# pabr/leansdr

Measured on AMD Instinct MI355X. Metric: IQ MSamples/s demodulated (leandvb QPSK 1/2), higher is better.
Workload: dtype f32; 1 GPU; BASELINE config 2: QPSK 1/2, Fs 240 MS/s cf32 (120 sps), device-resident endless stream; scaler(x75 fused) + fir_filter(N=313,D=30) + cstln_receiver(omega 4, linear sampler); fir_arith=LSDR_FIR_MFMA_BLK (f32 matrix pipe, block-polyphase; tolera…, batch_samples_per_capture=268369920, captures_per_gpu=1, rx_mode=tiled, parallelism=1 independent capture(s), 1 per GPU, no collectives, no RCCL

## Files before the change

### leansdr_amd/csrc/cstln_receiver.hip

```cpp
#include <cmath>
#include "capture_input.h"

namespace {

constexpr int kChunk = 128;
constexpr int kRrcLdsTaps = 1024;

#ifdef LSDR_RX_TRACE
__device__ unsigned long long g_rx_probe[8];
#define LSDR_RXP(i) { asm volatile("s_waitcnt vmcnt(0) lgkmcnt(0)" ::: "memory"); unsigned long long t__ = __builtin_amdgcn_s_memtime(); \
  asm volatile("s_waitcnt lgkmcnt(0)" ::: "memory"); \
  if (i > 0) rxp_acc[i] += t__ - rxp_t; else if (rxp_t) rxp_acc[4] += t__ - rxp_t; \
  if (i == 3) { rxp_acc[0] += 1; unsigned long long u__ = __builtin_amdgcn_s_memtime(); asm volatile("s_waitcnt lgkmcnt(0)" ::: "memory"); rxp_acc[5] += u__ - t__; t__ = u__; } \
  rxp_t = t__; }
#define LSDR_RXP_FLUSH { if (threadIdx.x == 0 && blockIdx.x == (gridDim.x > 1 ? 1u : 0u)) for (int k__ = 0; k__ < 6; ++k__) atomicAdd(&g_rx_probe[k__], rxp_acc[k__]); }
#else
#define LSDR_RXP(i)
#define LSDR_RXP_FLUSH
#endif
constexpr float kCstlnAmp = 75.0f;

struct __attribute__((aligned(8))) lut_entry {
  int16_t cost;
  uint8_t symbol;
// ... 430 lines not shown
        st.meas_count -= a.C.meas_decimation;
        rx_meas m; m.freqw = st.freqw; m.est_insp = st.est_insp; m.est_sp = st.est_sp; m.est_ep = st.est_ep; m.a = 0.f; m.tile = 0u;
        a.meas[sh_nm++] = m;
      }
    }
    pos += kChunk;
    __syncthreads();
    if (have_next) {
#pragma unroll
      for (int q = 0; q < 3; ++q)
        if (lane + 64 * q < span) buf[lane + 64 * q] = pre[q];
      for (int k = lane + 192; k < span; k += 64) buf[k] = src[pos + k];
    }
    __syncthreads();
  }
  if (lane == 0) {
    *a.state = st;
    a.counters[0] = pos; a.counters[1] = sh_nout; a.counters[2] = sh_nm; a.counters[3] = sh_nc;
  }
}


struct rx_state_dev;
__device__ __forceinline__ lsdr_softsymbol rx_relabel(lsdr_softsymbol v, const uint8_t *map) { v.symbol = map[v.symbol]; return v; }
__device__ __forceinline__ unsigned rx_symbol_of(lsdr_softsymbol v) { return v.symbol; }
__device__ __forceinline__ float fmod65536(float x);
__device__ __forceinline__ void rx_rotate_back(rx_state_dev *st, unsigned rot, float quad);
__device__ __forceinline__ float rx_freq_tap(const rx_state_dev *st) { return st->freqw / 65536; }
#include "rx_tiling.h"
typedef rx_tile_info_t<lsdr_softsymbol> rx_tile_info;

__device__ __forceinline__ void rx_rotate_back(rx_state_dev *st, unsigned rot, float quad) {
  st->phase = fmod65536(st->phase - rot * quad);
}

struct rx_tiled_args {
  const void *in;
  unsigned long long total_chunks;
  unsigned first_chunks, tile_chunks, warm_chunks;
  unsigned n_tiles;
  unsigned lanes_per_wave;
  unsigned dbg;
  unsigned stage_stride;
  lsdr_softsymbol *stage;
  lsdr_softsymbol *wstage;
  unsigned wstride;
  rx_tile_info *info;
  unsigned *hstage;
  unsigned long long hpitch;
  rx_tile_info_h *hinfo;
  rx_ema_map *ema;
  rx_ema_map *ema_wave;
  const rx_state_dev *state;
  rx_state_dev *state_next;
  rx_meas *meas;
  unsigned long long meas_base;
  float2 *cstln;
  rx_consts C;
  rx_tables T;
};

__device__ __forceinline__ void rx_tile_meas(const rx_tiled_args &a, unsigned long long c, unsigned tile, float freqw,
                                             const rx_ema_map &m) {
  const unsigned long long md = a.C.meas_decimation;
  const unsigned long long before = (a.meas_base + c * kChunk) / md, after = (a.meas_base + (c + 1) * kChunk) / md;
  const unsigned long long first_m = a.meas_base / md;
  for (unsigned long long q = before; q < after; ++q) {
    rx_meas mm; mm.freqw = freqw; mm.a = m.a; mm.est_insp = m.bi; mm.est_sp = m.bs; mm.est_ep = m.be; mm.tile = tile;
    a.meas[q - first_m] = mm;
  }
}

template <int SAMP, int FMT, bool HARD, bool SOFT_T = false>
__device__ __forceinline__ void rx_tile_exact(const rx_tiled_args &a, float in_scale = 1.0f, unsigned in_flip = 0u) {
  typename in_stream<FMT>::type src = in_make<FMT>(a.in);
  in_conv(src, in_scale, in_flip);
  unsigned long long c1 = a.first_chunks;
  if (c1 > a.total_chunks) c1 = a.total_chunks;
  rx_state_dev s = *a.state;
  rx_tile_info ti;
  ti.has_pre = 0; ti.pre.cost = 0; ti.pre.symbol = 0; ti.pre.pad = 0; ti.n_warm = 0;
  ti.mu_begin = s.mu; ti.phase_begin = s.phase;
  lsdr_softsymbol *po = a.stage;
  unsigned cnt = 0;
  unsigned hacc = 0, htail = 0;
  auto emit = [&](lsdr_softsymbol ss) {
    if (HARD) {
      hacc = (hacc << 2) | (ss.symbol & 3u); htail = (htail << 2) | (ss.symbol & 3u);
      if (SOFT_T) { po[(unsigned long long)cnt * a.hpitch] = ss; ++cnt; }
      else if ((++cnt & 15u) == 0) a.hstage[(unsigned long long)((cnt >> 4) - 1) * a.hpitch] = hacc;
    } else {
      po[cnt++] = ss;
    }
  };
  rx_ema_map m; m.a = 0.f; m.bi = s.est_insp; m.bs = s.est_sp; m.be = s.est_ep;
  for (unsigned long long c = 0; c < c1; ++c) {
    if (SAMP == 1) s.samp_freqw = s.freqw;
    if (SAMP == 2) {
      int ph = s.update_freq_phase - 128;
      if (ph <= 0) {
        const float f = s.freqw / a.C.subsampling;
        const int N = a.C.ncoeffs;
        for (int i = 0; i < N; ++i) {
          const float2 e = ld_uniform::expi(a.T, trig_index(-f * (i - N / 2)));
          const float cc = a.T.coeffs[i];
          a.T.shifted[i] = make_float2(e.x * cc, e.y * cc);
        }
        ph = N * 16;
      }
      s.update_freq_phase = ph;
    }
    bool wrote;
    rx_chunk<SAMP, ld_uniform>(a.T, a.C, s, src + c * kChunk, emit, a.cstln ? a.cstln + c : nullptr, &wrote);
    if (a.cstln && !wrote) a.cstln[c] = make_float2(__builtin_nanf(""), __builtin_nanf(""));
    m.bi = s.est_insp; m.bs = s.est_sp; m.be = s.est_ep;
    if (a.meas) rx_tile_meas(a, c, 0u, s.freqw, m);
  }
  ti.mu_end = s.mu; ti.phase_end = s.phase; ti.count = cnt;
  if (HARD) {
    if (!SOFT_T && (cnt & 15u)) a.hstage[(unsigned long long)(cnt >> 4) * a.hpitch] = hacc << (2 * (16 - (cnt & 15u)));
    rx_tile_info_h th;
    th.mu_begin = ti.mu_begin; th.phase_begin = ti.phase_begin; th.mu_end = ti.mu_end; th.phase_end = ti.phase_end;
    th.count = cnt; th.has_pre = 0; th.n_warm = 0; th.warm_tail = 0; th.body_tail = htail;
    a.hinfo[0] = th;
  } else {
    a.info[0] = ti;
  }
  { rx_ema_map id; id.a = 1.f; id.bi = id.bs = id.be = 0.f; a.ema[0] = id; }
  a.ema_wave[0] = m;
  if (a.n_tiles == 1) {
    s.meas_count = (a.meas_base + a.total_chunks * kChunk) % a.C.meas_decimation;
    *a.state_next = s;
  }
}

template <int FMT> struct rx_stage;
template <> struct rx_stage<LSDR_IN_CU8> {
  static constexpr int kStage = 64;
  static constexpr int kStageMargin = 16;
  static constexpr int kBps = 2;
  static constexpr int kRowBytes = kBps * (kStage + kStageMargin) + 16;
  static constexpr int kWindow = 8;
};
template <> struct rx_stage<LSDR_IN_CF32> {
  static constexpr int kStage = 16;
  static constexpr int kStageMargin = 1;
  static constexpr int kBps = 8;
  static constexpr int kRowBytes = kBps * (kStage + kStageMargin) + 8;
  static constexpr int kWindow = 16;
};
static_assert(rx_stage<LSDR_IN_CU8>::kRowBytes % 16 == 0 && rx_stage<LSDR_IN_CF32>::kRowBytes % 16 == 0, "stage geometry");
static_assert(kChunk % rx_stage<LSDR_IN_CU8>::kStage == 0 && kChunk % rx_stage<LSDR_IN_CF32>::kStage == 0, "stage geometry");
typedef __attribute__((address_space(3))) void *rx_lds_ptr;

constexpr int kEstSpan = 512;
template <typename SRC>
__device__ __forceinline__ float rx_wave_timing(const SRC &src, long long first, long long end, float omega, int lane, float *quality) {
  float cr = 0.f, sr = 0.f, pw = 0.f;
  const float w = 1.0f / omega;
#pragma unroll
  for (int i = 0; i < kEstSpan / 64; ++i) {
    const int idx = i * 64 + lane;
    if (first + idx < end) {
      const float2 x = src[first + idx];
      const float hann = 0.5f - 0.5f * __builtin_amdgcn_cosf((float)idx * (1.0f / kEstSpan));
      const float p = (x.x * x.x + x.y * x.y) * hann;
      const float rev = (float)idx * w;
      const float fr = rev - __builtin_floorf(rev);
      cr += p * __builtin_amdgcn_cosf(fr); sr += p * __builtin_amdgcn_sinf(fr); pw += p;
    }
  }
#pragma unroll
  for (int d = 32; d >= 1; d >>= 1) { cr += __shfl_xor(cr, d, 64); sr += __shfl_xor(sr, d, 64); pw += __shfl_xor(pw, d, 64); }
  *quality = pw > 0.f ? __builtin_sqrtf(cr * cr + sr * sr) / pw : 0.f;
  float rev = atan2f(sr, cr) * 0.15915494f;
  rev -= __builtin_floorf(rev);
  return rev * omega;
}

template <int SAMP, bool ARITH, int FMT, bool LDS, bool HARD>
__device__ __forceinline__ void rx_tile_tol(const rx_tiled_args &a, unsigned j0, int lane, char *lds) {
  const bool valid = lane < (int)a.lanes_per_wave && j0 + (unsigned)lane < a.n_tiles;
  const rx_consts &C = a.C;
  const bool rrc_lds = SAMP == 2 && C.ncoeffs <= kRrcLdsTaps;
  float est_first = 0.f, est_step = 0.f;
  bool est_ok = false;
  unsigned est_j0 = j0;
  if (SAMP != 2 && C.omega >= 2.0f && (a.lanes_per_wave == 32u || a.lanes_per_wave == 64u)) {
    const long long end = (long long)a.total_chunks * kChunk + (SAMP == 1 ? 1 : 0);
    const typename in_stream<FMT>::type all = in_make<FMT>(a.in);
    for (unsigned g = 0; g < a.lanes_per_wave / 32u; ++g) {
      const unsigned jf = j0 + 32u * g;
      if (jf >= a.n_tiles) break;
      const unsigned jl = jf + 31u < a.n_tiles - 1 ? jf + 31u : a.n_tiles - 1;
      const long long wsf = ((long long)a.first_chunks + (long long)(jf - 1) * a.tile_chunks - a.warm_chunks) * kChunk;
      const long long wsl = wsf + (long long)(jl - jf) * a.tile_chunks * kChunk;
      float q0 = 0.f, q1 = 0.f, step = 0.f;
      const float t0 = rx_wave_timing(all, wsf, end, C.omega, lane, &q0);
      const bool ok = q0 > 0.02f && wsf + kEstSpan <= end;
      if (ok && jl > jf && wsl + kEstSpan <= end) {
        const float t1 = rx_wave_timing(all, wsl, end, C.omega, lane, &q1);
        if (q1 > 0.02f) {
          const double span = (double)(wsl - wsf), om = (double)C.omega;
          double pred = (double)t0 - span; pred -= om * __builtin_floor(pred / om);
          float d = t1 - (float)pred;
          d -= C.omega * __builtin_rintf(d / C.omega);
          step = d / (float)(jl - jf);
        }
      }
      if ((unsigned)lane / 32u == g || a.lanes_per_wave == 32u) { est_first = t0; est_step = step; est_ok = ok; est_j0 = jf; }
    }
  }
  if (!LDS && !valid) return;
  const unsigned j = valid ? j0 + (unsigned)lane : j0;
  const unsigned long long c0 = a.first_chunks + (unsigned long long)(j - 1) * a.tile_chunks;
  unsigned long long c1 = c0 + a.tile_chunks;
  if (c1 > a.total_chunks) c1 = a.total_chunks;
  const unsigned long long cb = c0 - a.warm_chunks;
  const int nwarm = (int)a.warm_chunks, nchunks = valid ? (int)(c1 - cb) : 0;
  const int wave_chunks = LDS ? nwarm + (int)a.tile_chunks : nchunks;
  const int ra = SAMP == 1 ? 1 : (SAMP == 2 ? C.ncoeffs - 1 : 0);
  const int n_last = nchunks * kChunk - 1 + ra;
  const typename in_stream<FMT>::type base = in_make<FMT>(a.in) + cb * kChunk;

  typedef rx_stage<FMT> ST;
  constexpr int kStage = ST::kStage, kRowBytes = ST::kRowBytes, kStageLoads = ST::kRowBytes / 16;
  const char *row = nullptr;
  int delta = 0;
  __amdgpu_buffer_rsrc_t rsrc;
  unsigned src_off[LDS ? kStageLoads : 1];
  if (LDS) {
    const unsigned long long addr = (unsigned long long)a.in;
    delta = (int)(addr & 15ull);
    const unsigned long long cb0 = a.first_chunks + (unsigned long long)(j0 - 1) * a.tile_chunks - a.warm_chunks;
    const unsigned long long org = FMT == LSDR_IN_CU8 ? 0ull : cb0;
    const unsigned long long bytes = (((a.total_chunks - org) * kChunk + (unsigned)ra) * (unsigned)ST::kBps + (unsigned)delta + 15ull) & ~15ull;
    rsrc = __builtin_amdgcn_make_buffer_rsrc(const_cast<char *>(reinterpret_cast<const char *>(a.in)) + org * (kChunk * ST::kBps) - delta, 0,
                                             (int)(bytes > 0xffffffffull ? 0xffffffffu : (unsigned)bytes), 0x00020000);
    row = lds + lane * kRowBytes;
#pragma unroll
    for (int q = 0; q < kStageLoads; ++q) {
      const unsigned f = (unsigned)q * 1024u + (unsigned)lane * 16u, r = f / (unsigned)kRowBytes, col = f - r * (unsigned)kRowBytes;
      const unsigned long long tile_byte = (cb0 - org + (unsigned long long)r * a.tile_chunks) * (kChunk * (unsigned long long)ST::kBps);
      src_off[q] = (j0 + r < a.n_tiles && tile_byte + col < 0xfff00000ull) ? (unsigned)(tile_byte + col) : 0xfffffff0u;
    }
  }

  const rx_state_dev *S = a.state;
  float freqw = S->freqw, agc = S->agc_gain, est_insp = S->est_insp, est_sp = S->est_sp, est_ep = S->est_ep;
  const float min_f = S->min_freqw, max_f = S->max_freqw;
  float fwin = 65536.0f / C.omega / 2048.0f;
  if (fwin < 8.f) fwin = 8.f;
  const float f_lo = freqw - fwin, f_hi = freqw + fwin;
  float mu = 0.f, phase = 0.f;
  {
    const double ws = (double)cb * kChunk - (double)S->mu, om = (double)C.omega;
    const double r = ws - om * __builtin_floor(ws / om);
    mu = (float)(r > 0.0 ? om - r : 0.0);
    if (est_ok) {
      const double off = (double)(j - est_j0) * a.tile_chunks * kChunk;
      double t = (double)est_first + (double)est_step * (double)(j - est_j0) - off;
      t -= om * __builtin_floor(t / om);
      float dm = (float)t - mu;
      dm -= C.omega * __builtin_rintf(dm / C.omega);
      if (__builtin_fabsf(dm) > 0.33f) mu = (float)t;
    }
    if (!(mu >= 0.f && mu < C.omega)) mu = 0.f;
  }
  float h0pr = 0.f, h0pi = 0.f, h0cr = 0.f, h0ci = 0.f, h1pr = 0.f, h1pi = 0.f, h1cr = 0.f, h1ci = 0.f;
  float h2pr = 0.f, h2pi = 0.f, h2cr = 0.f, h2ci = 0.f;
  const float kk = C.kest, k1 = 1 - C.kest;
  const float acq_alpha = C.acq_alpha, freq_alpha = C.freq_alpha, acq_gain_mu = C.acq_gain_mu, gain_mu = C.gain_mu;
  const float freq_beta = C.freq_beta, omega = C.omega;
  const int acq_syms = C.acq_syms;
  rx_ema_map m; m.a = 1.f; m.bi = 0.f; m.bs = 0.f; m.be = 0.f;

  rx_tile_info ti;
  ti.has_pre = 0; ti.pre.cost = 0; ti.pre.symbol = 0; ti.pre.pad = 0; ti.n_warm = 0;
  ti.mu_begin = ti.phase_begin = 0.f;
  unsigned last = 0;
  unsigned *const po = reinterpret_cast<unsigned *>(a.stage + (unsigned long long)j * a.stage_stride);
  unsigned *const pw = reinterpret_cast<unsigned *>(a.wstage + (unsigned long long)j * a.wstride);
  unsigned *const pw0 = reinterpret_cast<unsigned *>(a.wstage + (unsigned long long)j0 * a.wstride);
  unsigned cnt = 0, got = 0;
  unsigned hacc = 0, htail = 0, hwarm = 0, hnwarm = 0, hcnt = 0;
  unsigned q0 = 0, q1 = 0, q2 = 0, q3 = 0, qn = 0;
  unsigned *bp = po;
  const bool quads = !HARD && !(a.dbg & 1u);
  unsigned *const hcol = HARD ? a.hstage + j : nullptr;

  int n = 0;
  rx_window<FMT> win;
  if (!LDS) {
    win.load(base, 0, n_last);
    if (!HARD) *pw = 0u;
  } else {
    win.wn = -16;
  }
  for (int ci = 0; ci < wave_chunks; ++ci) {
    const bool active = !LDS || ci < nchunks;
    const bool body = ci >= nwarm, lastwarm = ci + 1 == nwarm;
    const int cend = (ci + 1) * kChunk;
    if (active && ci == nwarm) {
      ti.mu_begin = mu; ti.phase_begin = phase;
      ti.pre.cost = (int16_t)(last & 0xffffu); ti.pre.symbol = (uint8_t)(last >> 16); ti.has_pre = got ? 1u : 0u;
      hwarm = htail; hnwarm = got < 16u ? got : 16u;
    }
    const float samp_freqw = freqw;
    unsigned *dp = body ? po + cnt : (lastwarm ? pw : pw0);
    unsigned keep = (body || lastwarm) ? 1u : 0u;
    if (a.dbg & 1u) { dp = pw0; keep = 0u; }
    bool had = false;
    float2 sg = make_float2(0.f, 0.f), sv = make_float2(0.f, 0.f);
    int pt_re = 0, pt_im = 0;
    unsigned nsym = 0;
    auto skip = [&]() {
      if (!(mu < 1.f)) {
        const int rem = cend - n;
        int k = (int)mu;
        if (k < 1 || k > rem) k = rem;
        mu -= (float)k; n += k; phase += (float)k * freqw;
      }
    };
    if (active) skip();
#pragma unroll 1
    for (int sb = 0; sb < (LDS ? kChunk / kStage : 1); ++sb) {
      const int s0 = ci * kChunk + sb * kStage;
      const int send = LDS ? s0 + kStage : cend;
      auto lds_window = [&](rx_window<FMT> &wd, int i) {
        int bo = ST::kBps * (i - s0) + delta;
        bo = bo < 0 ? 0 : (bo > kRowBytes - ST::kWindow ? kRowBytes - ST::kWindow : bo);
        rx_window_lds(wd, row, bo, delta, s0);
      };
      if (LDS) {
        const unsigned soff = (unsigned)__builtin_amdgcn_readfirstlane(s0 * ST::kBps);
#pragma unroll
        for (int q = 0; q < kStageLoads; ++q)
          __builtin_amdgcn_raw_ptr_buffer_load_lds(rsrc, (rx_lds_ptr)(size_t)(unsigned)(unsigned long long)(lds + q * 1024), 16, src_off[q], soff, 0, 0);
        __builtin_amdgcn_s_waitcnt(0x0F70);
        asm volatile("" ::: "memory");
        if (active && n < send && (FMT == LSDR_IN_CF32 || !win.covers(n))) lds_window(win, n);
      }
      while (active && n < send) {
        if (SAMP != 2 && !win.covers(n) && !(a.dbg & 2u)) {
          if (LDS) lds_window(win, n);
          else {
            win.load(base, n, n_last);
            __builtin_amdgcn_s_waitcnt(0x0F70);
          }
        }
        float2 p0, p1;
        win.get(n, p0, p1);
        const float2 sx0 = cmul(p0, ld_hwtrig::expi(a.T, trig_index(-phase)));
        if (SAMP == 2) {
          float2 acc = make_float2(0.f, 0.f);
          const int SS = C.subsampling, N = C.ncoeffs;
          int px = n;
          int pc = (int)((1 - mu) * SS);
          auto tap = [&](int i) -> float2 { return rrc_lds ? reinterpret_cast<const float2 *>(lds)[i] : a.T.shifted_tol[i]; };
          if (FMT == LSDR_IN_CF32) {
            for (; pc + SS < N; pc += 2 * SS, px += 2) {
              const float4 xx = *reinterpret_cast<const float4 *>(reinterpret_cast<const float2 *>(base.p) + px);
              const float2 t0 = cmul(tap(pc), make_float2(xx.x, xx.y));
              acc.x += t0.x; acc.y += t0.y;
              const float2 t1 = cmul(tap(pc + SS), make_float2(xx.z, xx.w));
              acc.x += t1.x; acc.y += t1.y;
            }
          }
          for (; pc < N; pc += SS, ++px) {
            const float2 tt = cmul(tap(pc), base[px]);
            acc.x += tt.x; acc.y += tt.y;
          }
          sg = cmul(ld_hwtrig::expi(a.T, trig_index(-phase)), acc);
        } else if (SAMP == 1) {
          const float2 sx1 = cmul(p1, ld_hwtrig::expi(a.T, trig_index(-(phase + samp_freqw))));
          const float k0 = 1 - mu;
          sg = make_float2(sx0.x * k0 + sx1.x * mu, sx0.y * k0 + sx1.y * mu);
        } else {
          sg = sx0;
        }
        sv = make_float2(sg.x * agc, sg.y * agc);
        uint2 raw;
        if (!ARITH) raw = *reinterpret_cast<const uint2 *>(a.T.lut + lut_index(sv.x, sv.y));
        int lo = (int)(mu + omega - 0.1f);
        lo = lo < 1 ? 1 : lo;
        rx_window<FMT> nxt;
        if (LDS) lds_window(nxt, n + lo);
        else if (a.dbg & 2u) { nxt = win; nxt.wn = n + lo; }
        else nxt.load(base, n + lo, n_last);
        lut_entry e;
        if (ARITH) {
          float hi = sv.x, hq = sv.y;
          lut_halve(hi, hq);
          const qpsk_decision qd = qpsk_decide((int)hi, (int)hq);
          e.cost = (int16_t)qd.cost; e.symbol = (uint8_t)qd.symbol; e.zero = 0;
          e.phase_error = (int16_t)qd.phase_error; e.pt_re = (int8_t)qd.pt_re; e.pt_im = (int8_t)qd.pt_im;
          raw.x = ((unsigned)qd.cost & 0xffffu) | (qd.symbol << 16);
        } else {
          e = lut_unpack(raw.x, raw.y);
        }
        if (HARD) {
          const unsigned hs = (raw.x >> 16) & 3u;
          htail = (htail << 2) | hs;
          if (body) {
            hacc = (hacc << 2) | hs;
            if ((++hcnt & 15u) == 0) hcol[(unsigned long long)((hcnt >> 4) - 1) * a.hpitch] = hacc;
          }
        } else if (quads && body) {
          q0 = q1; q1 = q2; q2 = q3; q3 = raw.x;
          if (++qn == 4u) {
            *reinterpret_cast<uint4 *>(bp) = make_uint4(q0, q1, q2, q3);
            bp += 4; qn = 0;
          }
        } else {
          *dp = raw.x; dp += keep;
        }
        last = raw.x;
        ++nsym;
        const bool acq = (int)(got + nsym) <= acq_syms && !body;
        phase += e.phase_error * (acq ? acq_alpha : freq_alpha);
        freqw += e.phase_error * freq_beta;
        freqw = freqw < f_lo ? f_lo : freqw; freqw = freqw > f_hi ? f_hi : freqw;
        h2pr = h1pr; h2pi = h1pi; h2cr = h1cr; h2ci = h1ci;
        h1pr = h0pr; h1pi = h0pi; h1cr = h0cr; h1ci = h0ci;
        h0pr = sv.x; h0pi = sv.y;
        pt_re = e.pt_re; pt_im = e.pt_im;
        had = true;
        h0cr = (float)pt_re; h0ci = (float)pt_im;
        const float muerr = ((h0pr - h2pr) * h1cr + (h0pi - h2pi) * h1ci) - ((h0cr - h2cr) * h1pr + (h0ci - h2ci) * h1pi);
        float mucorr = muerr * (acq ? acq_gain_mu : gain_mu);
        mucorr = mucorr < -0.1f ? -0.1f : mucorr; mucorr = mucorr > 0.1f ? 0.1f : mucorr;
        mu += mucorr;
        mu += omega;
        mu -= 1.f; phase += freqw; ++n;
        win = nxt;
        skip();
      }
    }
    if (active) {
      phase = fmod65536(phase);
      if (had) {
        const float insp = sg.x * sg.x + sg.y * sg.y;
        est_insp = insp * kk + est_insp * k1;
        if (est_insp) agc = kCstlnAmp / __builtin_sqrtf(est_insp);
        const float evr = sv.x - pt_re, evi = sv.y - pt_im;
        float sig_power, ev_power;
        if (C.nsymbols == 2) {
          const float sig_real = (float)((double)(pt_re + pt_im) * 0.707);
          const float ev_real = (float)((double)(evr + evi) * 0.707);
          sig_power = sig_real * sig_real; ev_power = ev_real * ev_real;
        } else {
          sig_power = (float)(pt_re * pt_re + pt_im * pt_im);
          ev_power = evr * evr + evi * evi;
        }
        est_sp = sig_power * kk + est_sp * k1;
        est_ep = ev_power * kk + est_ep * k1;
        if (body) {
          m.a *= k1;
          m.bi = insp * kk + m.bi * k1; m.bs = sig_power * kk + m.bs * k1; m.be = ev_power * kk + m.be * k1;
        }
      }
      if (!C.allow_drift) {
        if (freqw < min_f || freqw > max_f) freqw = (max_f + min_f) / 2;
      }
      if (body) cnt += nsym; else got += nsym;
      if (lastwarm) ti.n_warm = nsym;
      if (body && a.meas) rx_tile_meas(a, cb + (unsigned long long)ci, j, freqw, m);
      if (body && a.cstln) a.cstln[cb + (unsigned long long)ci] = had ? sv : make_float2(__builtin_nanf(""), __builtin_nanf(""));
    }
  }
  ti.mu_end = mu; ti.phase_end = phase; ti.count = cnt;
  if (quads && qn) {
    const uint4 v = qn == 1u ? make_uint4(q3, 0u, 0u, 0u) : (qn == 2u ? make_uint4(q2, q3, 0u, 0u) : make_uint4(q1, q2, q3, 0u));
    *reinterpret_cast<uint4 *>(bp) = v;
  }
  if (valid) {
    if (HARD) {
      if (hcnt & 15u) hcol[(unsigned long long)(hcnt >> 4) * a.hpitch] = hacc << (2 * (16 - (hcnt & 15u)));
      rx_tile_info_h th;
      th.mu_begin = ti.mu_begin; th.phase_begin = ti.phase_begin; th.mu_end = mu; th.phase_end = phase;
      th.count = cnt; th.has_pre = ti.has_pre; th.n_warm = hnwarm; th.warm_tail = hwarm; th.body_tail = htail;
      a.hinfo[j] = th;
    } else {
      a.info[j] = ti;
    }
  }
  {
    rx_ema_map inc = m;
    const int gl = lane & 31;
#pragma unroll
    for (int d = 1; d < 32; d <<= 1) {
      rx_ema_map o;
// ... 173 lines not shown
    nout += cnt;
    s.meas_count += kChunk;
    while (s.meas_count >= a.C.meas_decimation) s.meas_count -= a.C.meas_decimation;
  }
  if (quads && (nout & 3ull)) {
    unsigned *pu = reinterpret_cast<unsigned *>(po);
    const unsigned r = (unsigned)(nout & 3ull);
    if (r == 1u) pu[nout - 1] = q3;
    else if (r == 2u) { pu[nout - 2] = q2; pu[nout - 1] = q3; }
    else { pu[nout - 3] = q1; pu[nout - 2] = q2; pu[nout - 1] = q3; }
  }
  a.states[sidx] = s;
  a.produced[sidx] = nout;
}

#include "notch_detect.h"
#include "rxb_device.h"

}

struct lsdr_rx {
  lsdr_ctx *ctx;
  lsdr_rx_cfg cfg;
  std::vector<float> coeffs;
  lsdr::cstln_tables tabs;
  float omega, min_omega, max_omega;
  rx_state_dev st;
  rx_state_dev st_initial;
  bool st_dirty_host;
  float2 *d_trig;
  lut_entry *d_lut;
  float *d_coeffs;
  float2 *d_shifted, *d_shifted_tol;
  rx_state_dev *d_state;
  unsigned long long *d_counters;
  rx_meas *d_meas; size_t meas_cap;
  float2 *d_cstln; size_t cstln_cap;
  lsdr_softsymbol *d_stage; size_t stage_cap;
  lsdr_softsymbol *d_wstage; size_t wstage_cap;
  unsigned *d_hstage; size_t hstage_cap;
  rx_tile_info_h *d_hinfo;
  size_t out_sym_offset;
  bool time_on; hipEvent_t tev0[8], tev1[8]; bool tev_set[8]; double time_ms; unsigned time_n;
  rx_tile_info *d_info; rx_tile_fix *d_fix; size_t tiles_cap;
  rx_ema_map *d_ema;
  rx_ema_map *d_ema_wave;
  rx_state_dev *d_state_next;
  rx_state_dev *h_snap;
  static constexpr unsigned kSnapSlots = 4;
  uint8_t *d_relabel;
  struct rx_seam_result *d_seam;
  struct rx_seam_part *d_part;
  std::vector<uint8_t> relabel;
  unsigned last_tiles, last_dup, last_miss, last_badseam;
  static const int kRing = 8;
  struct rx_seam_result *h_res;
  struct rx_seam_result *h_res_dev;
  hipEvent_t ev[kRing];
  unsigned ring_tiles[kRing];
  int ring_head, ring_count;
  float retired_freq_tap;
  bool st_stale_host;
  bool qpsk_arith;
  unsigned arith_max_dpe;
};

static void rx_state_export(const rx_state_dev &s, lsdr_rx_state *st) {
  st->mu = s.mu; st->phase = s.phase; st->freqw = s.freqw; st->agc_gain = s.agc_gain;
  st->est_insp = s.est_insp; st->est_sp = s.est_sp; st->est_ep = s.est_ep;
  st->freq_tap = s.freqw / 65536;
  st->min_freqw = s.min_freqw; st->max_freqw = s.max_freqw;
  st->meas_count = s.meas_count;
  memcpy(st->hist, s.hist, sizeof(st->hist));
}

static void rx_update_freq_limits(lsdr_rx *r, bool have_cstln) {
  int n = 4;
  if (have_cstln) {
    switch (r->tabs.nsymbols) {
      case 2: n = 2; break;
      case 4: n = 4; break;
      case 8: n = 8; break;
      case 16: n = 12; break;
      case 32: n = 16; break;
      default: n = 4; break;
    }
  }
  r->st.min_freqw = r->st.freqw - 65536 / r->max_omega / n / 2;
  r->st.max_freqw = r->st.freqw + 65536 / r->max_omega / n / 2;
}
static void rx_set_omega(lsdr_rx *r, float omega, bool have_cstln) {
  float tol = (float)10e-6;
  r->omega = omega;
  r->min_omega = omega * (1 - tol);
  r->max_omega = omega * (1 + tol);
  rx_update_freq_limits(r, have_cstln);
}
static void rx_set_freq(lsdr_rx *r, float freq, bool have_cstln) {
  r->st.freqw = freq * 65536;
  rx_update_freq_limits(r, have_cstln);
}

static int rx_push_state(lsdr_rx *r) {
  if (!r->st_dirty_host) return LSDR_OK;
  LSDR_HIP(hipMemcpyAsync(r->d_state, &r->st, sizeof(rx_state_dev), hipMemcpyHostToDevice, r->ctx->stream));
  LSDR_HIP(hipStreamSynchronize(r->ctx->stream));
  r->st_dirty_host = false;
  return LSDR_OK;
}

static void rx_fill_consts(const lsdr_rx *r, rx_consts &C, rx_tables &T) {
  C.omega = r->omega;
  C.freq_alpha = (float)0.04;
  C.freq_beta = (float)(0.0012 / (double)r->omega * (double)r->cfg.pll_adjustment);
  C.gain_mu = (float)(0.02 / (double)(kCstlnAmp * kCstlnAmp) * 2);
  C.kest = r->cfg.kest;
  C.allow_drift = r->cfg.allow_drift;
  C.nsymbols = r->tabs.nsymbols;
  C.meas_decimation = r->cfg.meas_decimation;
  C.ncoeffs = r->cfg.ncoeffs;
  C.subsampling = r->cfg.subsampling;
  {
    const char *e;
    C.acq_syms = (e = getenv("LSDR_RX_ACQ_SYMS")) ? atoi(e) : 0;
    C.acq_alpha = C.freq_alpha * ((e = getenv("LSDR_RX_ACQ_ALPHA")) ? (float)atof(e) : 1.f);
    C.acq_gain_mu = C.gain_mu * ((e = getenv("LSDR_RX_ACQ_MU")) ? (float)atof(e) : 1.f);
  }
  T.trig = r->d_trig; T.lut = r->d_lut; T.coeffs = r->d_coeffs; T.shifted = r->d_shifted; T.shifted_tol = r->d_shifted_tol;
}

static int rx_pull_state(lsdr_rx *r) {
  if (!r->st_stale_host) return LSDR_OK;
  LSDR_HIP(hipMemcpyAsync(&r->st, r->d_state, sizeof(rx_state_dev), hipMemcpyDeviceToHost, r->ctx->stream));
  LSDR_HIP(hipStreamSynchronize(r->ctx->stream));
  r->st_stale_host = false;
  return LSDR_OK;
}

struct rx_plan {
  rx_tiled_args a;
  lsdr_softsymbol *out;
  size_t chunks, nm;
  unsigned n_tiles, blocks, lpw, stage_stride, sym_per_chunk;
  unsigned long long hpitch, meas_base, md;
  bool want_meas, want_cstln, use_lds, hard;
  int slot;
};

struct rx_hooks {
  bool no_lds_set; int no_lds;
  unsigned long long lds_span;
  int lanes;
  bool prio;
  unsigned dbg; bool skip;
};
static const rx_hooks &rx_env() {
  static const rx_hooks h = [] {
    rx_hooks v;
    const char *e = getenv("LSDR_RX_NO_LDS");
    v.no_lds_set = e != nullptr; v.no_lds = e ? atoi(e) : 0;
    v.lds_span = (e = getenv("LSDR_RX_LDS_SPAN")) ? strtoull(e, nullptr, 0) : 0xfff00000ull;
    v.lanes = (e = getenv("LSDR_RX_LANES")) ? atoi(e) : 0;
    v.prio = (e = getenv("LSDR_RX_PRIO")) && atoi(e);
    v.dbg = (e = LSDR_MEASURE_ENV("LSDR_RX_DBG")) ? (unsigned)atoi(e) & 3u : 0u;
    v.skip = LSDR_MEASURE_ENV("LSDR_RX_SKIP") != nullptr;
    return v;
  }();
  return h;
}

template <typename T>
static int rx_grow(T **buf, size_t *cap, size_t need) {
  if (*cap >= need) return LSDR_OK;
  (void)hipFree(*buf); *buf = nullptr; *cap = 0;
  LSDR_HIP(hipMalloc((void **)buf, need * sizeof(T)));
  *cap = need;
  return LSDR_OK;
}

static int rx_tiled_plan(lsdr_rx *r, unsigned share, const void *in, size_t n_in, lsdr_softsymbol *out, size_t cap_out,
                         bool want_meas, size_t meas_cap, size_t cstln_cap, rx_plan *P) {
  lsdr_ctx *c = r->ctx;
  LSDR_HIP(hipSetDevice(c->device));
  P->out = out; P->chunks = 0; P->nm = 0; P->n_tiles = 0;
  if (r->ring_count == lsdr_rx::kRing) { lsdr_set_error("cstln_receiver: too many queued runs (lsdr_rx_wait first)"); return LSDR_E_ARG; }
  const int ra = lsdr_rx_readahead(r);
  unsigned Wc = r->cfg.tile_warmup ? r->cfg.tile_warmup / kChunk : (unsigned)((64.0f * r->omega + kChunk - 1) / kChunk);
  if (!r->cfg.tile_warmup && Wc < 1) Wc = 1;
  unsigned Lc = r->cfg.tile_len ? r->cfg.tile_len / kChunk : 2 * Wc;
  LSDR_ARG(Lc >= 1 && Wc >= 1);
  const unsigned sym_per_chunk = (unsigned)(kChunk / (r->omega - 0.1f)) + 2;
  size_t chunks = n_in >= (size_t)(kChunk + ra) ? (n_in - ra) / kChunk : 0;
  if ((size_t)(sym_per_chunk + 1) * chunks > cap_out) chunks = cap_out / (sym_per_chunk + 1);
  const bool want_cstln = cstln_cap > 0;
  if (want_cstln && chunks > cstln_cap) chunks = cstln_cap;
  const rx_hooks &H = rx_env();
  const bool cu8 = r->cfg.in_format == LSDR_IN_CU8;
  bool use_lds = r->cfg.sampler != LSDR_SAMP_FIR && (cu8 ? H.no_lds != 1 && r->omega <= 8.f : H.no_lds == 0);
  if (use_lds && cu8 && !H.no_lds_set) {
    const unsigned long long max_samples = (H.lds_span - 64) / 2;
    if ((unsigned long long)chunks * kChunk + (unsigned)ra > max_samples) chunks = (size_t)((max_samples - (unsigned)ra) / kChunk);
  }
  const int slot = (r->ring_head + r->ring_count) % lsdr_rx::kRing;
  P->slot = slot; P->chunks = chunks; P->want_meas = want_meas; P->want_cstln = want_cstln;
  if (!chunks) return LSDR_OK;
  const unsigned first = Wc;
  unsigned n_tiles = 1;
  if (chunks > first) n_tiles += (unsigned)((chunks - first + Lc - 1) / Lc);
  const unsigned stage_stride = ((first > Lc ? first : Lc) * sym_per_chunk + 3u + 4u) & ~3u;

  const bool hard = r->cfg.out_format == LSDR_SYM_HARD2;
  const unsigned hstride = stage_stride / 16 + 2;
  const unsigned long long hpitch = ((unsigned long long)n_tiles + 63) & ~63ull;
  const unsigned long long md = r->cfg.meas_decimation;
  const unsigned long long meas_base = r->st.meas_count;
  const size_t nm = (size_t)((meas_base + chunks * kChunk) / md - meas_base / md);
  P->nm = nm; P->meas_base = meas_base; P->md = md;
  if (want_meas && nm > meas_cap) { lsdr_set_error("cstln_receiver(tiled): measurement buffers too small"); return LSDR_E_ARG; }
  const size_t need_hstage = hard ? (size_t)hpitch * hstride : 0, need_stage = hard ? 0 : (size_t)n_tiles * stage_stride,
               need_wstage = hard ? 0 : (size_t)n_tiles * sym_per_chunk, need_meas = want_meas ? nm + 1 : 0, need_cstln = want_cstln ? chunks : 0;
  if (r->tiles_cap < n_tiles || r->hstage_cap < need_hstage || r->stage_cap < need_stage || r->wstage_cap < need_wstage ||
      r->meas_cap < need_meas || r->cstln_cap < need_cstln) {
    LSDR_HIP(hipStreamSynchronize(c->stream));
  }
  if (r->tiles_cap < n_tiles) {
    (void)hipFree(r->d_info); (void)hipFree(r->d_fix); (void)hipFree(r->d_part); (void)hipFree(r->d_ema);
    LSDR_HIP(hipMalloc((void **)&r->d_ema, n_tiles * sizeof(rx_ema_map)));
    (void)hipFree(r->d_ema_wave);
    LSDR_HIP(hipMalloc((void **)&r->d_ema_wave, ((size_t)n_tiles + 1) * sizeof(rx_ema_map)));
    LSDR_HIP(hipMalloc((void **)&r->d_part, ((n_tiles + kSeamBlock - 1) / kSeamBlock) * sizeof(rx_seam_part)));
    LSDR_HIP(hipMalloc((void **)&r->d_info, n_tiles * sizeof(rx_tile_info)));
    LSDR_HIP(hipMalloc((void **)&r->d_fix, n_tiles * sizeof(rx_tile_fix)));
    (void)hipFree(r->d_hinfo); r->d_hinfo = nullptr;
    if (hard) LSDR_HIP(hipMalloc((void **)&r->d_hinfo, n_tiles * sizeof(rx_tile_info_h)));
    r->tiles_cap = n_tiles;
  }
  LSDR_TRY(rx_grow(&r->d_hstage, &r->hstage_cap, need_hstage));
  LSDR_TRY(rx_grow(&r->d_stage, &r->stage_cap, need_stage));
  LSDR_TRY(rx_grow(&r->d_wstage, &r->wstage_cap, need_wstage));
  LSDR_TRY(rx_grow(&r->d_meas, &r->meas_cap, need_meas));
  LSDR_TRY(rx_grow(&r->d_cstln, &r->cstln_cap, need_cstln));
  int rc = rx_push_state(r);
  if (rc) return rc;

  rx_tiled_args &a = P->a;
  a.in = in;
  a.total_chunks = chunks;
  a.first_chunks = first; a.tile_chunks = Lc; a.warm_chunks = Wc;
  a.n_tiles = n_tiles;
  a.stage_stride = stage_stride;
  a.stage = r->d_stage;
  a.wstage = r->d_wstage; a.wstride = sym_per_chunk;
  a.hstage = r->d_hstage; a.hpitch = hpitch; a.hinfo = r->d_hinfo;
  a.info = r->d_info;
  a.ema = r->d_ema;
  a.ema_wave = r->d_ema_wave;
  a.state = r->d_state;
  a.state_next = r->d_state_next;
  a.meas = want_meas ? r->d_meas : nullptr;
  a.meas_base = meas_base;
  a.cstln = want_cstln ? r->d_cstln : nullptr;
  rx_fill_consts(r, a.C, a.T);
  const bool lanes_ok = H.lanes >= 1 && (H.lanes <= 32 || H.lanes == 64);
  const unsigned lpw = lanes_ok ? (unsigned)H.lanes : (unsigned long long)n_tiles * share > 12288ull ? 64u : 32u;
  a.lanes_per_wave = lpw;
  a.dbg = H.dbg | (H.prio ? 4u : 0u);
  if (!cu8) use_lds = use_lds && lpw == 64 && (unsigned long long)n_tiles * share <= 65536ull && ((unsigned long long)in & 7ull) == 0;
  const unsigned blocks = 1 + (n_tiles - 1 + lpw - 1) / lpw;
  P->n_tiles = n_tiles; P->blocks = blocks; P->lpw = lpw; P->stage_stride = stage_stride; P->sym_per_chunk = sym_per_chunk;
  P->hpitch = hpitch; P->hard = hard;
  if (hard && !(use_lds && cu8)) { lsdr_set_error("cstln_receiver: LSDR_SYM_HARD2 needs cu8 input with the nearest or linear sampler"); return LSDR_E_UNSUPPORTED; }
  if (hard && (float)Lc * kChunk / (r->omega + 0.1f) < 34.f) {
    lsdr_set_error("cstln_receiver: LSDR_SYM_HARD2 needs tiles of at least 34 symbols (tile_len %u samples at omega %.2f)", Lc * kChunk, (double)r->omega);
    return LSDR_E_ARG;
  }
  P->use_lds = use_lds;
  return LSDR_OK;
}

typedef void (*rx_tiles_kernel_t)(rx_tiled_multi);
template <int S, bool A>
static rx_tiles_kernel_t rx_tiles_of(bool cu8, bool use_lds, bool hard) {
  constexpr bool L = S != 2;
  if (hard) return k_rx_tiles<S, A, LSDR_IN_CU8, L, L>;
  if (use_lds) return cu8 ? k_rx_tiles<S, A, LSDR_IN_CU8, L, false> : k_rx_tiles<S, A, LSDR_IN_CF32, L, false>;
  return cu8 ? k_rx_tiles<S, A, LSDR_IN_CU8, false, false> : k_rx_tiles<S, A, LSDR_IN_CF32, false, false>;
}
static rx_tiles_kernel_t rx_kernel_tiles(int sampler, bool arith, bool cu8, bool use_lds, bool hard) {
  switch (sampler) {
    case LSDR_SAMP_NEAREST: return arith ? rx_tiles_of<0, true>(cu8, use_lds, hard) : rx_tiles_of<0, false>(cu8, use_lds, hard);
    case LSDR_SAMP_LINEAR: return arith ? rx_tiles_of<1, true>(cu8, use_lds, hard) : rx_tiles_of<1, false>(cu8, use_lds, hard);
  }
  return arith ? rx_tiles_of<2, true>(cu8, use_lds, hard) : rx_tiles_of<2, false>(cu8, use_lds, hard);
}

static int rx_tiled_launch(lsdr_rx *const *rs, const rx_plan *P, unsigned n) {
  lsdr_rx *r = rs[0];
  lsdr_ctx *c = r->ctx;
  const unsigned n_tiles = P[0].n_tiles, lpw = P[0].lpw, stage_stride = P[0].stage_stride;
  const int slot = P[0].slot;
  const bool timed = n == 1 && r->time_on;
  rx_tiled_multi tm;
  rx_seam_multi sm;
  rx_ema_multi em;
  for (unsigned i = 0; i < (unsigned)kRxMulti; ++i) {
    const unsigned k = i < n ? i : 0;
    tm.a[i] = P[k].a;
    sm.c[i] = rx_seam_rec{rs[k]->d_info, rs[k]->d_fix, rs[k]->d_part, rs[k]->d_stage, rs[k]->d_wstage, P[k].out, rs[k]->d_state,
                          rs[k]->h_res_dev + P[k].slot};
    em.c[i] = rx_ema_rec{rs[k]->d_ema_wave, rs[k]->d_ema, rs[k]->d_state_next, rs[k]->d_state};
  }
  if (n == 1 && r->cfg.sampler == LSDR_SAMP_FIR)
    hipLaunchKernelGGL(k_rx_fir_refresh, dim3(1), dim3(256), 0, c->stream, (const rx_state_dev *)r->d_state, (const float2 *)r->d_trig,
                       (const float *)r->d_coeffs, r->cfg.ncoeffs, r->cfg.subsampling, r->d_shifted_tol);
  if (timed) { LSDR_HIP(hipEventRecord(r->tev0[slot], c->stream)); }
  hipLaunchKernelGGL(rx_kernel_tiles(r->cfg.sampler, r->qpsk_arith, r->cfg.in_format == LSDR_IN_CU8, P[0].use_lds, P[0].hard),
                     dim3(P[0].blocks, n), dim3(64), 0, c->stream, tm);
  if (n == 1) r->tev_set[slot] = timed;
  if (timed) { LSDR_HIP(hipEventRecord(r->tev1[slot], c->stream)); }
  LSDR_HIP(hipGetLastError());
  const int R = r->tabs.nrotations;
  const float quad = 65536.0f / R;
  const bool meas = n == 1 && P[0].want_meas;
  rx_meas *const d_meas = meas ? r->d_meas : nullptr;
  const unsigned n_meas = meas ? (unsigned)P[0].nm : 0u;
  if (P[0].hard) {
    hipLaunchKernelGGL(k_rx_ema, dim3(1), dim3(kEmaThreads), 0, c->stream, (const rx_ema_map *)r->d_ema_wave, rx_ema_groups(n_tiles, lpw),
                       (const rx_ema_map *)r->d_ema, n_tiles, rx_ema_group(lpw), (const rx_state_dev *)r->d_state_next, r->d_state, d_meas, n_meas);
    hipLaunchKernelGGL(k_rx_seam_h, dim3((n_tiles + kSeamBlock - 1) / kSeamBlock), dim3(kSeamBlock), 0, c->stream,
                       (const rx_tile_info_h *)r->d_hinfo, r->d_fix, n_tiles, r->omega, R, quad, r->d_part, (const uint8_t *)r->d_relabel);
    hipLaunchKernelGGL((k_rx_compact_h<rx_state_dev>), dim3((n_tiles + 63) / 64), dim3(64), 0, c->stream, (const unsigned *)r->d_hstage, P[0].hpitch,
                       (const rx_tile_info_h *)r->d_hinfo, (const rx_tile_fix *)r->d_fix, (const rx_seam_part *)r->d_part,
                       (const uint8_t *)r->d_relabel, n_tiles, R, quad, reinterpret_cast<unsigned *>(P[0].out),
                       (unsigned long long)r->out_sym_offset, r->d_state, r->h_res_dev + slot);
  } else {
    hipLaunchKernelGGL(k_rx_seam_ema_multi, dim3((n_tiles + kSeamBlock - 1) / kSeamBlock + 1, n), dim3(kSeamBlock), 0, c->stream, sm, em, n_tiles,
                       r->omega, R, quad, stage_stride, P[0].sym_per_chunk, (const uint8_t *)r->d_relabel, rx_ema_groups(n_tiles, lpw),
                       rx_ema_group(lpw), d_meas, n_meas);
    hipLaunchKernelGGL(k_rx_compact_multi, dim3((n_tiles + kCompactTiles - 1) / kCompactTiles, n), dim3(64), 0, c->stream, sm, n_tiles, R, quad,
                       stage_stride, (const uint8_t *)r->d_relabel);
  }
  LSDR_HIP(hipGetLastError());
  return LSDR_OK;
}

static int rx_tiled_commit(lsdr_rx *r, const rx_plan &P, hipStream_t stream, size_t *consumed) {
  const int slot = P.slot;
  if (!P.chunks) {
    r->h_res[slot].total = 0; r->h_res[slot].rot_final = 0; r->h_res[slot].ndup = r->h_res[slot].nmiss = r->h_res[slot].nbad = 0;
    r->h_res[slot].freq_tap = r->retired_freq_tap;
    r->ring_tiles[slot] = 0; r->tev_set[slot] = false;
    LSDR_HIP(hipEventRecord(r->ev[slot], stream));
    ++r->ring_count;
    *consumed = 0;
    return LSDR_OK;
  }
  LSDR_HIP(hipEventRecord(r->ev[slot], stream));
  r->ring_tiles[slot] = P.n_tiles;
  ++r->ring_count;
  r->st_stale_host = true;
  r->st.meas_count = (P.meas_base + P.chunks * kChunk) % P.md;
  *consumed = P.chunks * kChunk;
  return LSDR_OK;
}

static int rx_tiled_enqueue(lsdr_rx *r, const void *in, size_t n_in, lsdr_softsymbol *out, size_t cap_out,
                            size_t *consumed, bool want_meas, size_t meas_cap, size_t *nm_out, size_t cstln_cap = 0,
                            size_t *chunks_out = nullptr) {
  *consumed = 0;
  if (nm_out) *nm_out = 0;
  rx_plan P;
  LSDR_TRY(rx_tiled_plan(r, 1u, in, n_in, out, cap_out, want_meas, meas_cap, cstln_cap, &P));
  if (chunks_out) *chunks_out = P.chunks;
  if (P.chunks) LSDR_TRY(rx_tiled_launch(&r, &P, 1));
  LSDR_TRY(rx_tiled_commit(r, P, r->ctx->stream, consumed));
  if (nm_out) *nm_out = P.nm;
  return LSDR_OK;
}

static int rx_tiled_enqueue_multi(lsdr_rx *const *rs, unsigned n, const void *const *ins, size_t n_in, lsdr_softsymbol *const *outs,
                                  size_t cap_out, size_t *consumed) {
  for (unsigned i = 0; i < n; ++i) consumed[i] = 0;
  bool alike = n >= 2 && n <= (unsigned)kRxMulti;
  for (unsigned i = 1; i < n && alike; ++i) {
    const lsdr_rx *a = rs[0], *b = rs[i];
    alike = a->ctx == b->ctx && a->cfg.sampler == b->cfg.sampler && a->cfg.in_format == b->cfg.in_format &&
            a->cfg.out_format == b->cfg.out_format && a->cfg.tile_len == b->cfg.tile_len && a->cfg.tile_warmup == b->cfg.tile_warmup &&
            a->cfg.cstln == b->cfg.cstln && a->omega == b->omega && a->qpsk_arith == b->qpsk_arith && a->cfg.ncoeffs == b->cfg.ncoeffs &&
            a->cfg.subsampling == b->cfg.subsampling && a->tabs.nrotations == b->tabs.nrotations && a->time_on == b->time_on;
  }
  if (alike) alike = rs[0]->cfg.out_format != LSDR_SYM_HARD2 && rs[0]->cfg.sampler != LSDR_SAMP_FIR && !rs[0]->time_on;
  std::vector<rx_plan> Pv(n);
  rx_plan *P = Pv.data();
  for (unsigned i = 0; i < n; ++i) LSDR_TRY(rx_tiled_plan(rs[i], alike ? n : 1u, ins[i], n_in, outs[i], cap_out, false, 0, 0, &P[i]));
  for (unsigned i = 1; i < n && alike; ++i)
    alike = P[i].chunks == P[0].chunks && P[i].n_tiles == P[0].n_tiles && P[i].blocks == P[0].blocks && P[i].lpw == P[0].lpw &&
            P[i].stage_stride == P[0].stage_stride && P[i].use_lds == P[0].use_lds;
  if (!alike || !P[0].chunks) {
    for (unsigned i = 0; i < n; ++i) {
      if (P[i].chunks) LSDR_TRY(rx_tiled_launch(&rs[i], &P[i], 1));
      LSDR_TRY(rx_tiled_commit(rs[i], P[i], rs[i]->ctx->stream, &consumed[i]));
    }
    return LSDR_OK;
  }
  if (!rx_env().skip) LSDR_TRY(rx_tiled_launch(rs, P, n));
  for (unsigned i = 0; i < n; ++i) LSDR_TRY(rx_tiled_commit(rs[i], P[i], rs[0]->ctx->stream, &consumed[i]));
  return LSDR_OK;
}

static int rx_tiled_wait(lsdr_rx *r, size_t *produced) {
  if (!r->ring_count) { lsdr_set_error("cstln_receiver: no queued run"); return LSDR_E_ARG; }
  const int slot = r->ring_head;
  LSDR_HIP(hipEventSynchronize(r->ev[slot]));
  if (r->tev_set[slot]) {
    float ms = 0.f;
    if (hipEventElapsedTime(&ms, r->tev0[slot], r->tev1[slot]) == hipSuccess) { r->time_ms += ms; ++r->time_n; }
    r->tev_set[slot] = false;
  }
  const rx_seam_result sr = r->h_res[slot];
// ... 467 lines not shown
```

Before: 684,900 MS/s.

## Prefetch LDS stage rows into registers and batch timing-estimate loads

The per-stage direct-to-LDS buffer loads followed by a full waitcnt are replaced by a register double-buffer. Each stage writes the rows loaded earlier into LDS, then issues buffer loads for the next stage so global latency overlaps with the current stage's compute. The initial timing estimation is also split into a load phase and a compute phase, with loads for both lane groups issued together, and the first stage prefetch is started before it. This costs extra VGPRs, which may reduce occupancy, and keeps the old synchronous path behind an env flag.

```diff
diff --git a/leansdr_amd/csrc/cstln_receiver.hip b/leansdr_amd/csrc/cstln_receiver.hip
--- a/leansdr_amd/csrc/cstln_receiver.hip
+++ b/leansdr_amd/csrc/cstln_receiver.hip
@@ -606,17 +606,26 @@
 static_assert(rx_stage<LSDR_IN_CU8>::kRowBytes % 16 == 0 && rx_stage<LSDR_IN_CF32>::kRowBytes % 16 == 0, "stage geometry");
 static_assert(kChunk % rx_stage<LSDR_IN_CU8>::kStage == 0 && kChunk % rx_stage<LSDR_IN_CF32>::kStage == 0, "stage geometry");
 typedef __attribute__((address_space(3))) void *rx_lds_ptr;
+typedef unsigned rx_u4 __attribute__((ext_vector_type(4)));
 
 constexpr int kEstSpan = 512;
+struct rx_timing_samples { float2 x[kEstSpan / 64]; };
 template <typename SRC>
-__device__ __forceinline__ float rx_wave_timing(const SRC &src, long long first, long long end, float omega, int lane, float *quality) {
+__device__ __forceinline__ void rx_wave_timing_load(const SRC &src, long long first, long long end, int lane, rx_timing_samples &s) {
+#pragma unroll
+  for (int i = 0; i < kEstSpan / 64; ++i) {
+    const long long k = first + (i * 64 + lane);
+    s.x[i] = src[k < end ? k : end - 1];
+  }
+}
+__device__ __forceinline__ float rx_wave_timing(const rx_timing_samples &s, long long first, long long end, float omega, int lane, float *quality) {
   float cr = 0.f, sr = 0.f, pw = 0.f;
   const float w = 1.0f / omega;
 #pragma unroll
   for (int i = 0; i < kEstSpan / 64; ++i) {
     const int idx = i * 64 + lane;
     if (first + idx < end) {
-      const float2 x = src[first + idx];
+      const float2 x = s.x[i];
       const float hann = 0.5f - 0.5f * __builtin_amdgcn_cosf((float)idx * (1.0f / kEstSpan));
       const float p = (x.x * x.x + x.y * x.y) * hann;
       const float rev = (float)idx * w;
@@ -637,45 +646,7 @@
   const bool valid = lane < (int)a.lanes_per_wave && j0 + (unsigned)lane < a.n_tiles;
   const rx_consts &C = a.C;
   const bool rrc_lds = SAMP == 2 && C.ncoeffs <= kRrcLdsTaps;
-  float est_first = 0.f, est_step = 0.f;
-  bool est_ok = false;
-  unsigned est_j0 = j0;
-  if (SAMP != 2 && C.omega >= 2.0f && (a.lanes_per_wave == 32u || a.lanes_per_wave == 64u)) {
-    const long long end = (long long)a.total_chunks * kChunk + (SAMP == 1 ? 1 : 0);
-    const typename in_stream<FMT>::type all = in_make<FMT>(a.in);
-    for (unsigned g = 0; g < a.lanes_per_wave / 32u; ++g) {
-      const unsigned jf = j0 + 32u * g;
-      if (jf >= a.n_tiles) break;
-      const unsigned jl = jf + 31u < a.n_tiles - 1 ? jf + 31u : a.n_tiles - 1;
-      const long long wsf = ((long long)a.first_chunks + (long long)(jf - 1) * a.tile_chunks - a.warm_chunks) * kChunk;
-      const long long wsl = wsf + (long long)(jl - jf) * a.tile_chunks * kChunk;
-      float q0 = 0.f, q1 = 0.f, step = 0.f;
-      const float t0 = rx_wave_timing(all, wsf, end, C.omega, lane, &q0);
-      const bool ok = q0 > 0.02f && wsf + kEstSpan <= end;
-      if (ok && jl > jf && wsl + kEstSpan <= end) {
-        const float t1 = rx_wave_timing(all, wsl, end, C.omega, lane, &q1);
-        if (q1 > 0.02f) {
-          const double span = (double)(wsl - wsf), om = (double)C.omega;
-          double pred = (double)t0 - span; pred -= om * __builtin_floor(pred / om);
-          float d = t1 - (float)pred;
-          d -= C.omega * __builtin_rintf(d / C.omega);
-          step = d / (float)(jl - jf);
-        }
-      }
-      if ((unsigned)lane / 32u == g || a.lanes_per_wave == 32u) { est_first = t0; est_step = step; est_ok = ok; est_j0 = jf; }
-    }
-  }
-  if (!LDS && !valid) return;
-  const unsigned j = valid ? j0 + (unsigned)lane : j0;
-  const unsigned long long c0 = a.first_chunks + (unsigned long long)(j - 1) * a.tile_chunks;
-  unsigned long long c1 = c0 + a.tile_chunks;
-  if (c1 > a.total_chunks) c1 = a.total_chunks;
-  const unsigned long long cb = c0 - a.warm_chunks;
-  const int nwarm = (int)a.warm_chunks, nchunks = valid ? (int)(c1 - cb) : 0;
-  const int wave_chunks = LDS ? nwarm + (int)a.tile_chunks : nchunks;
   const int ra = SAMP == 1 ? 1 : (SAMP == 2 ? C.ncoeffs - 1 : 0);
-  const int n_last = nchunks * kChunk - 1 + ra;
-  const typename in_stream<FMT>::type base = in_make<FMT>(a.in) + cb * kChunk;
 
   typedef rx_stage<FMT> ST;
   constexpr int kStage = ST::kStage, kRowBytes = ST::kRowBytes, kStageLoads = ST::kRowBytes / 16;
@@ -683,6 +654,9 @@
   int delta = 0;
   __amdgpu_buffer_rsrc_t rsrc;
   unsigned src_off[LDS ? kStageLoads : 1];
+  const bool stage_sync = LDS && (a.dbg & 8u);
+  const int stage_end = LDS ? (int)(a.warm_chunks + a.tile_chunks) * kChunk : 0;
+  rx_u4 pre[LDS ? kStageLoads : 1];
   if (LDS) {
     const unsigned long long addr = (unsigned long long)a.in;
     delta = (int)(addr & 15ull);
@@ -698,7 +672,68 @@
       const unsigned long long tile_byte = (cb0 - org + (unsigned long long)r * a.tile_chunks) * (kChunk * (unsigned long long)ST::kBps);
       src_off[q] = (j0 + r < a.n_tiles && tile_byte + col < 0xfff00000ull) ? (unsigned)(tile_byte + col) : 0xfffffff0u;
     }
-  }
+#pragma unroll
+    for (int q = 0; q < kStageLoads; ++q) pre[q] = rx_u4{0u, 0u, 0u, 0u};
+    if (!stage_sync) {
+#pragma unroll
+      for (int q = 0; q < kStageLoads; ++q) pre[q] = __builtin_amdgcn_raw_buffer_load_b128(rsrc, (int)src_off[q], 0, 0);
+    }
+  }
+  float est_first = 0.f, est_step = 0.f;
+  bool est_ok = false;
+  unsigned est_j0 = j0;
+  if (SAMP != 2 && C.omega >= 2.0f && (a.lanes_per_wave == 32u || a.lanes_per_wave == 64u)) {
+    const long long end = (long long)a.total_chunks * kChunk + (SAMP == 1 ? 1 : 0);
+    const typename in_stream<FMT>::type all = in_make<FMT>(a.in);
+    const unsigned n_groups = a.lanes_per_wave / 32u;
+    constexpr unsigned kRound = LDS ? 2u : 1u;
+    rx_timing_samples ts[2][2];
+#pragma unroll
+    for (unsigned g0 = 0; g0 < 2u; g0 += kRound) {
+#pragma unroll
+      for (unsigned g = g0; g < g0 + kRound; ++g) {
+        const unsigned jf = j0 + 32u * g;
+        if (g >= n_groups || jf >= a.n_tiles) break;
+        const unsigned jl = jf + 31u < a.n_tiles - 1 ? jf + 31u : a.n_tiles - 1;
+        const long long wsf = ((long long)a.first_chunks + (long long)(jf - 1) * a.tile_chunks - a.warm_chunks) * kChunk;
+        const long long wsl = wsf + (long long)(jl - jf) * a.tile_chunks * kChunk;
+        rx_wave_timing_load(all, wsf, end, lane, ts[g][0]);
+        if (jl > jf && wsl + kEstSpan <= end) rx_wave_timing_load(all, wsl, end, lane, ts[g][1]);
+      }
+#pragma unroll
+      for (unsigned g = g0; g < g0 + kRound; ++g) {
+        const unsigned jf = j0 + 32u * g;
+        if (g >= n_groups || jf >= a.n_tiles) break;
+        const unsigned jl = jf + 31u < a.n_tiles - 1 ? jf + 31u : a.n_tiles - 1;
+        const long long wsf = ((long long)a.first_chunks + (long long)(jf - 1) * a.tile_chunks - a.warm_chunks) * kChunk;
+        const long long wsl = wsf + (long long)(jl - jf) * a.tile_chunks * kChunk;
+        float q0 = 0.f, q1 = 0.f, step = 0.f;
+        const float t0 = rx_wave_timing(ts[g][0], wsf, end, C.omega, lane, &q0);
+        const bool ok = q0 > 0.02f && wsf + kEstSpan <= end;
+        if (ok && jl > jf && wsl + kEstSpan <= end) {
+          const float t1 = rx_wave_timing(ts[g][1], wsl, end, C.omega, lane, &q1);
+          if (q1 > 0.02f) {
+            const double span = (double)(wsl - wsf), om = (double)C.omega;
+            double pred = (double)t0 - span; pred -= om * __builtin_floor(pred / om);
+            float d = t1 - (float)pred;
+            d -= C.omega * __builtin_rintf(d / C.omega);
+            step = d / (float)(jl - jf);
+          }
+        }
+        if ((unsigned)lane / 32u == g || a.lanes_per_wave == 32u) { est_first = t0; est_step = step; est_ok = ok; est_j0 = jf; }
+      }
+    }
+  }
+  if (!LDS && !valid) return;
+  const unsigned j = valid ? j0 + (unsigned)lane : j0;
+  const unsigned long long c0 = a.first_chunks + (unsigned long long)(j - 1) * a.tile_chunks;
+  unsigned long long c1 = c0 + a.tile_chunks;
+  if (c1 > a.total_chunks) c1 = a.total_chunks;
+  const unsigned long long cb = c0 - a.warm_chunks;
+  const int nwarm = (int)a.warm_chunks, nchunks = valid ? (int)(c1 - cb) : 0;
+  const int wave_chunks = LDS ? nwarm + (int)a.tile_chunks : nchunks;
+  const int n_last = nchunks * kChunk - 1 + ra;
+  const typename in_stream<FMT>::type base = in_make<FMT>(a.in) + cb * kChunk;
 
   const rx_state_dev *S = a.state;
   float freqw = S->freqw, agc = S->agc_gain, est_insp = S->est_insp, est_sp = S->est_sp, est_ep = S->est_ep;
@@ -788,10 +823,20 @@
       };
       if (LDS) {
         const unsigned soff = (unsigned)__builtin_amdgcn_readfirstlane(s0 * ST::kBps);
+        if (stage_sync) {
 #pragma unroll
-        for (int q = 0; q < kStageLoads; ++q)
-          __builtin_amdgcn_raw_ptr_buffer_load_lds(rsrc, (rx_lds_ptr)(size_t)(unsigned)(unsigned long long)(lds + q * 1024), 16, src_off[q], soff, 0, 0);
-        __builtin_amdgcn_s_waitcnt(0x0F70);
+          for (int q = 0; q < kStageLoads; ++q)
+            __builtin_amdgcn_raw_ptr_buffer_load_lds(rsrc, (rx_lds_ptr)(size_t)(unsigned)(unsigned long long)(lds + q * 1024), 16, src_off[q], soff, 0, 0);
+          __builtin_amdgcn_s_waitcnt(0x0F70);
+        } else {
+#pragma unroll
+          for (int q = 0; q < kStageLoads; ++q) *reinterpret_cast<rx_u4 *>(lds + q * 1024 + lane * 16) = pre[q];
+          if (s0 + kStage < stage_end) {
+#pragma unroll
+            for (int q = 0; q < kStageLoads; ++q)
+              pre[q] = __builtin_amdgcn_raw_buffer_load_b128(rsrc, (int)src_off[q], (int)(soff + (unsigned)(kStage * ST::kBps)), 0);
+          }
+        }
         asm volatile("" ::: "memory");
         if (active && n < send && (FMT == LSDR_IN_CF32 || !win.covers(n))) lds_window(win, n);
       }
@@ -1271,6 +1316,7 @@
   unsigned long long lds_span;
   int lanes;
   bool prio;
+  bool stage_sync;
   unsigned dbg; bool skip;
 };
 static const rx_hooks &rx_env() {
@@ -1281,6 +1327,7 @@
     v.lds_span = (e = getenv("LSDR_RX_LDS_SPAN")) ? strtoull(e, nullptr, 0) : 0xfff00000ull;
     v.lanes = (e = getenv("LSDR_RX_LANES")) ? atoi(e) : 0;
     v.prio = (e = getenv("LSDR_RX_PRIO")) && atoi(e);
+    v.stage_sync = (e = getenv("LSDR_RX_STAGE_SYNC")) && atoi(e);
     v.dbg = (e = LSDR_MEASURE_ENV("LSDR_RX_DBG")) ? (unsigned)atoi(e) & 3u : 0u;
     v.skip = LSDR_MEASURE_ENV("LSDR_RX_SKIP") != nullptr;
     return v;
@@ -1383,7 +1430,7 @@
   const bool lanes_ok = H.lanes >= 1 && (H.lanes <= 32 || H.lanes == 64);
   const unsigned lpw = lanes_ok ? (unsigned)H.lanes : (unsigned long long)n_tiles * share > 12288ull ? 64u : 32u;
   a.lanes_per_wave = lpw;
-  a.dbg = H.dbg | (H.prio ? 4u : 0u);
+  a.dbg = H.dbg | (H.prio ? 4u : 0u) | (H.stage_sync ? 8u : 0u);
   if (!cu8) use_lds = use_lds && lpw == 64 && (unsigned long long)n_tiles * share <= 65536ull && ((unsigned long long)in & 7ull) == 0;
   const unsigned blocks = 1 + (n_tiles - 1 + lpw - 1) / lpw;
   P->n_tiles = n_tiles; P->blocks = blocks; P->lpw = lpw; P->stage_stride = stage_stride; P->sym_per_chunk = sym_per_chunk;
```

After: 661,800 MS/s. 3.4% lower.
